# VinAIResearch/Point-Unet

Hardware: AMD Instinct MI355X
Metric: points_per_sec_forward (higher is better)
Workload: dtype f32

## Files before the change

point-unet_amd/csrc/common.h:

```cpp
#pragma once

#include <hip/hip_runtime.h>

#include <cstdarg>
#include <cstdint>
#include <cstdio>
#include <cstring>
#include <map>
#include <string>
#include <vector>

#include "../../include/pointseg.h"
#include "../../include/pointseg_train_ops.h"

namespace ps {

void set_error(const char* fmt, ...);

#define PS_HIP(expr)                                                                                  \
    do {                                                                                              \
        hipError_t _e = (expr);                                                                       \
        if (_e != hipSuccess) {                                                                       \
            ps::set_error("%s failed: %s (%s:%d)", #expr, hipGetErrorString(_e), __FILE__, __LINE__); \
            return PS_EHIP;                                                                           \
// ... 41 lines not shown
struct StageTimer {
    std::string name;
    std::vector<std::pair<hipEvent_t, hipEvent_t>> spans;
    int64_t launches = 0;
};

}

namespace ps {
struct PackJob {
    const float* w;
    int64_t sk, sn;
    int kind, cin, cout, ntb, p0, cblocks;
    void* out;
    int64_t total;
    bool same_key(const PackJob& o) const
    {
        return w == o.w && sk == o.sk && sn == o.sn && kind == o.kind && cin == o.cin && cout == o.cout && ntb == o.ntb && p0 == o.p0 && cblocks == o.cblocks;
    }
};
struct PackCache {
    int mode = 0;
    bool broken = false;
    size_t cursor = 0;
    std::vector<PackJob> jobs;
    std::vector<DevBuf> bufs;
    DevBuf table;
    int n_ops = 0, n_b3 = 0;
};
void* pack_slot(ps_context* c, const PackJob& key, size_t bytes, bool& launch);
int pack_cache_finish_recording(ps_context* c, PackCache& pc);
int pack_cache_replay(ps_context* c, PackCache& pc);
void pack_cache_clear(PackCache& pc);
int pack_batch_ops(ps_context* c, const PackJob* table, int n);
int pack_batch_b3(ps_context* c, const PackJob* table, int n);
}

namespace ps {
struct Tuning {
    double gemm32b_min_flops = 3e8;
    int gemm32b_rw = 0, gemm32b_cw = 0;
    bool gemm32_no_sk8 = false;
    bool att64_gemm = true;
    int att64_occ = 0;
    bool att_no_split = false;
    int64_t wgrad_b3_min_rows = 0;
    int64_t gemm_b3_min_rows = 0;
    int64_t wgrad_wgs = 512;
    bool bn_slice = false;
    bool inv_bucket = true;
    int inv_tile = 4096;
    bool gather_reduce_ordered = true;
    int maxpool_bwd_ordered = 1;
    bool train_act_bf16 = true;
    int train_att_gemm_split = -1;
    bool train_att_gemm = true;
    bool train_att128_fwd_gemm = true;
    bool train_fuse_residual = true;
    bool train_merge_syncbn = true;
    int convbn_max_c = 64;
    int convbn_rect_max = 1 << 30;
    bool wgrad_debug = false;
};
void tuning_from_env(Tuning& t);
}

struct ps_context {
    int device = 0;
    ps::Tuning tune;
    hipStream_t own_stream = nullptr;
    hipStream_t stream = nullptr;
    ps::Arena knn_arena;
    ps::Arena net_arena;
    ps::Arena sample_arena;
    ps::DevBuf stage_in;
    ps::DevBuf stage_out;
    ps::DevBuf red_ws;
    ps::DevBuf wgrad_ws;
    ps::PackCache* pack_cache = nullptr;
    ps::DevBuf ops_ring[4];
    int ops_ring_pos = 0;
    bool att_bf16x3 = true;
    bool regchain_b3 = true;
    bool att_lane = true;
    bool train_b3 = true;
    bool train_bf16 = false;
    bool train_act_bf16 = false;
    bool mid_lds_attr = false;
    size_t chain_lds_attr = 48 * 1024;
    std::map<const void*, size_t> regchain_lds_attr;
    bool deferred = false;
    int32_t* h_flags = nullptr;
    unsigned pending_mask = 0;
    uint64_t builds = 0;
    uint64_t samples = 0;
    uint64_t volume_samples = 0;
    uint64_t flag_serial[8] = {};
    int flag_kind[8] = {};
    int flag_slot = 0;
    int sticky_rc = 0;
    std::string sticky_msg;
    hipEvent_t flag_ev[8] = {};
    std::vector<char> host_ring[8];
    int ring_pos = 0;
    std::vector<char>& ring_next() { ring_pos = (ring_pos + 1) & 7; return host_ring[ring_pos]; }
    int check_deferred();
    int check_flag_slot(int s);
    int defer_status(const void* d_words, size_t bytes, int kind, uint64_t serial);
    struct PinSlot { void* p = nullptr; size_t cap = 0; hipEvent_t ev = nullptr; bool busy = false; };
    PinSlot pin[16];
    int pin_pos = 0;
    int upload_async(void* dst, const void* src, size_t bytes);
    bool timing = false;
    std::string timing_only;
    std::vector<ps::StageTimer> stages;
    std::vector<hipEvent_t> event_pool;
    size_t event_next = 0;
    int cur_stage = -1;
    hipEvent_t cur_start = nullptr;

    hipEvent_t get_event();
    void stage_begin(const char* name);
    void stage_end(int launches);
};

namespace ps {
struct Stage {
    ps_context* c;
    int n;
    bool on = false;
    Stage(ps_context* ctx, const char* name, int launches = 1) : c(ctx), n(launches)
    {
        on = c->timing && (c->timing_only.empty() || c->timing_only == name);
        if (on) c->stage_begin(name);
    }
    ~Stage()
    {
        if (on) c->stage_end(n);
    }
};

inline int ceil_div(int64_t a, int64_t b) { return (int)((a + b - 1) / b); }

inline uint64_t pyramid_stamp(const ps_pyramid* p)
{
    uint64_t h = 0x50535059524D4944ull ^ (uint64_t)p->B ^ ((uint64_t)p->K << 32) ^ ((uint64_t)p->num_layers << 48);
    for (int i = 0; i < p->num_layers && i < PS_MAX_LAYERS; ++i) {
        h = (h ^ (uint64_t)reinterpret_cast<uintptr_t>(p->sub_idx[i])) * 0x9E3779B97F4A7C15ull;
        h = (h ^ (uint64_t)reinterpret_cast<uintptr_t>(p->neigh_idx[i])) * 0x9E3779B97F4A7C15ull;
        h = (h ^ (uint64_t)reinterpret_cast<uintptr_t>(p->interp_idx[i])) * 0x9E3779B97F4A7C15ull;
        h = (h ^ (uint64_t)reinterpret_cast<uintptr_t>(p->order[i])) * 0x9E3779B97F4A7C15ull;
        h = (h ^ (uint64_t)p->n[i] ^ ((uint64_t)p->n[i + 1] << 32)) * 0x9E3779B97F4A7C15ull;
    }
    return h | 1ull;
}

int pool_max(ps_context* c, const float* feat, const int32_t* idx, const int32_t* order, float* out, int64_t B, int64_t n, int64_t m, int K, int ch,
             unsigned char* ties = nullptr);

int conv1x1(ps_context* c, const float* x, int64_t ldx, const float* w, bool w_transposed, const float* b, int64_t R, int64_t cin, int64_t cout, int leaky,
            int accumulate, float* y, int64_t ldy);
int att_bwd_split_impl(ps_context* c, const float* fl, int64_t ldl, const int32_t* idx, int64_t B, int64_t n_src, int64_t n_q, const float* fr,
                       int64_t ldr, const float* wfc, const float* dagg, int64_t K, int64_t d, float* dfl, int64_t lddl, float* dfr, int64_t lddr,
                       float* dwfc, float* dfl_rows, int64_t ld_rows, bool df_accum);
int random_sample_bwd_inv(ps_context* c, const float* dout, const float* out, const float* feature, const int32_t* pool_idx, const int32_t* offsets,
                          const int32_t* src, int64_t B, int64_t N, int64_t M, int64_t K, int64_t d, const uint8_t* ties, float* share_ws,
// ... 24 lines not shown
```

point-unet_amd/csrc/context.hip:

```cpp
#include "common.h"
#include "kdtree_build.h"

#include <cstdlib>

namespace ps {

static thread_local char g_err[512] = "";

void set_error(const char* fmt, ...)
{
    va_list ap;
    va_start(ap, fmt);
    vsnprintf(g_err, sizeof g_err, fmt, ap);
    va_end(ap);
}

int DevBuf::reserve(size_t bytes)
{
    if (bytes <= cap) return PS_OK;
    if (p) {
        hipError_t e = hipDeviceSynchronize();
        if (e != hipSuccess) {
            set_error("hipDeviceSynchronize failed: %s", hipGetErrorString(e));
            return PS_EHIP;
// ... 138 lines not shown
    }
    cur_start = get_event();
    if (cur_start) (void)hipEventRecord(cur_start, stream);
}

void ps_context::stage_end(int launches)
{
    hipEvent_t stop = get_event();
    if (stop) (void)hipEventRecord(stop, stream);
    if (cur_stage >= 0 && cur_start && stop) {
        stages[cur_stage].spans.push_back({cur_start, stop});
        stages[cur_stage].launches += launches;
    }
    cur_stage = -1;
}

extern "C" {

const char* ps_last_error(void) { return ps::g_err; }

}

namespace ps {
void tuning_from_env(Tuning& t)
{
#ifdef PS_TUNING_ENV
    auto num = [](const char* name, double& out) { const char* v = std::getenv(name); if (v && *v) { out = std::atof(v); return true; } return false; };
    auto flag = [&](const char* name, bool& b) { double v; if (num(name, v)) b = v != 0; };
    auto clampi = [&](const char* name, int64_t lo, int64_t hi, int64_t& x) { double v; if (num(name, v)) x = v < lo ? lo : (v > hi ? hi : (int64_t)v); };
    double v;
    if (num("PS_GEMM32B_MIN_FLOPS", v) && v >= 0) t.gemm32b_min_flops = v;
    if (num("PS_GEMM32B_RW", v) && (v == 1 || v == 2)) t.gemm32b_rw = (int)v;
    if (num("PS_GEMM32B_CW", v) && (v == 1 || v == 2)) t.gemm32b_cw = (int)v;
    t.gemm32_no_sk8 = std::getenv("PS_GEMM32_NO_SK8") != nullptr;
    flag("PS_ATT64_GEMM", t.att64_gemm);
    if (num("PS_ATT64_OCC", v) && (v == 1 || v == 2)) t.att64_occ = (int)v;
    t.att_no_split = std::getenv("PS_ATT_NO_SPLIT") != nullptr;
    clampi("PS_WGRAD_B3_MIN_ROWS", 0, 1ll << 40, t.wgrad_b3_min_rows);
    clampi("PS_GEMM_B3_MIN_ROWS", 0, 1ll << 40, t.gemm_b3_min_rows);
    clampi("PS_WGRAD_WGS", 64, 4096, t.wgrad_wgs);
    flag("PS_BN_SLICE", t.bn_slice);
    flag("PS_INV_BUCKET", t.inv_bucket);
    if (num("PS_INV_TILE", v) && (v == 4096 || v == 6144 || v == 8192)) t.inv_tile = (int)v;
    flag("PS_GATHER_REDUCE_ORDERED", t.gather_reduce_ordered);
    if (num("PS_MAXPOOL_BWD_ORDERED", v)) t.maxpool_bwd_ordered = v != 0;
    flag("PS_TRAIN_ACT_BF16", t.train_act_bf16);
    if (num("PS_TRAIN_ATT_GEMM_SPLIT", v)) t.train_att_gemm_split = v < 0 ? -1 : (v != 0);
    flag("PS_TRAIN_ATT_GEMM", t.train_att_gemm);
    flag("PS_TRAIN_ATT128_FWD_GEMM", t.train_att128_fwd_gemm);
    flag("PS_TRAIN_FUSE_RESIDUAL", t.train_fuse_residual);
    flag("PS_TRAIN_MERGE_SYNCBN", t.train_merge_syncbn);
    if (num("PS_CONVBN_MAX_C", v) && v >= 0 && v <= 4096) t.convbn_max_c = (int)v;
    if (num("PS_CONVBN_RECT_MAX", v) && v >= 0) t.convbn_rect_max = v > (double)(1 << 30) ? 1 << 30 : (int)v;
    t.wgrad_debug = std::getenv("PS_WGRAD_DEBUG") != nullptr;
#else
    (void)t;
#endif
}
}

extern "C" {
const char* ps_version(void) { return "pointseg-hip 0.1 gfx950"; }
int ps_abi_version(void) { return PS_ABI_VERSION; }

int ps_create(int device, ps_context** out)
{
    PS_CHECK(out != nullptr, "ps_create: out is NULL");
    int count = 0;
    PS_HIP(hipGetDeviceCount(&count));
    PS_CHECK(device >= 0 && device < count, "ps_create: device %d out of range (%d devices)", device, count);
    PS_HIP(hipSetDevice(device));
    ps_context* c = new ps_context();
    c->device = device;
    hipError_t e = hipStreamCreateWithFlags(&c->own_stream, hipStreamNonBlocking);
    if (e != hipSuccess) {
        delete c;
        ps::set_error("hipStreamCreate failed: %s", hipGetErrorString(e));
        return PS_EHIP;
    }
    c->stream = c->own_stream;
    ps::tuning_from_env(c->tune);
#ifdef PS_TUNING_ENV
    if (const char* v = std::getenv("PS_REGCHAIN_B3")) c->regchain_b3 = std::atof(v) != 0;
    if (const char* v = std::getenv("PS_ATT_LANE")) c->att_lane = std::atof(v) != 0;
#endif
    *out = c;
    return PS_OK;
}

int ps_destroy(ps_context* c)
{
    if (!c) return PS_OK;
    (void)hipSetDevice(c->device);
    (void)hipStreamSynchronize(c->stream);
    c->knn_arena.buf.release();
    c->net_arena.buf.release();
    c->sample_arena.buf.release();
    c->stage_in.release();
    c->stage_out.release();
    c->red_ws.release();
    c->wgrad_ws.release();
    for (auto& b : c->ops_ring) b.release();
    if (c->h_flags) (void)hipHostFree(c->h_flags);
    for (auto& e : c->flag_ev)
        if (e) (void)hipEventDestroy(e);
    for (auto& s : c->pin) {
        if (s.p) (void)hipHostFree(s.p);
        if (s.ev) (void)hipEventDestroy(s.ev);
    }
    for (hipEvent_t e : c->event_pool) (void)hipEventDestroy(e);
    if (c->own_stream) (void)hipStreamDestroy(c->own_stream);
    delete c;
    return PS_OK;
}

int ps_set_stream(ps_context* c, void* hip_stream)
{
    PS_CHECK(c != nullptr, "ps_set_stream: ctx is NULL");
    c->stream = static_cast<hipStream_t>(hip_stream);
    return PS_OK;
}

int ps_synchronize(ps_context* c)
{
    PS_CHECK(c != nullptr, "ps_synchronize: ctx is NULL");
    PS_HIP(hipStreamSynchronize(c->stream));
    return c->check_deferred();
}

int ps_set_train_gemm_bf16(ps_context* c, int on)
{
    PS_CHECK(c != nullptr, "ps_set_train_gemm_bf16: ctx is NULL");
    c->train_bf16 = on != 0;
    return PS_OK;
}

int ps_set_train_act_bf16(ps_context* c, int on)
{
    PS_CHECK(c != nullptr, "ps_set_train_act_bf16: ctx is NULL");
    c->train_act_bf16 = on != 0;
    return PS_OK;
}

int ps_set_train_gemm_b3(ps_context* c, int on)
{
    PS_CHECK(c != nullptr, "ps_set_train_gemm_b3: ctx is NULL");
    c->train_b3 = on != 0;
    return PS_OK;
}

int ps_set_att_bf16x3(ps_context* c, int on)
{
    PS_CHECK(c != nullptr, "ps_set_att_bf16x3: ctx is NULL");
    c->att_bf16x3 = on != 0;
    return PS_OK;
}

int ps_set_deferred_checks(ps_context* c, int on)
{
    PS_CHECK(c != nullptr, "ps_set_deferred_checks: ctx is NULL");
    if (on && !c->h_flags) PS_HIP(hipHostMalloc(reinterpret_cast<void**>(&c->h_flags), 8 * 4 * sizeof(int32_t)));
    if (!on && c->pending_mask) {
        PS_HIP(hipStreamSynchronize(c->stream));
        PS_TRY(c->check_deferred());
    }
    c->deferred = on != 0;
// ... 46 lines not shown
```

point-unet_amd/csrc/debug_hooks.h:

```cpp
#ifndef POINTSEG_DEBUG_H
#define POINTSEG_DEBUG_H
#include "../../include/pointseg.h"
#ifdef __cplusplus
extern "C" {
#endif
int ps_debug_knn_host(const float* support, const float* queries, int64_t B, int64_t n_support,
                      int64_t n_queries, int64_t K, int32_t* out_idx);
int ps_debug_kdtree_host(const float* support, int64_t n, int32_t* vind, int32_t* nodes, float* pts,
                         int32_t* root_depth, float* bbox);
int ps_debug_kdtree_device(ps_context* ctx, const float* support, int64_t n, int32_t* vind, int32_t* nodes,
                           float* pts, int32_t* root_depth, float* bbox);
#define PS_DEBUG_KDTREE_STATS 22
int ps_debug_kdtree_device_set(ps_context* ctx, const float* support, const int32_t* n, int64_t T, const int32_t* want_copy, int32_t* vind,
                               int32_t* nodes, float* pts, int32_t* fat, int32_t* root_depth, float* bbox, float* copy, int32_t* stats);
int ps_debug_pack_weights(const float* W, int cin, int cout, int ntb, float* out);
int ps_debug_pack_b3(const float* W, int cin, int cout, uint16_t* out);
int ps_debug_pack_b3_device(ps_context* ctx, const float* W, int cin, int cout, void* out);
int ps_debug_gemm32(ps_context* ctx, int split_bf16, const float* x1, int ld1, int c1, const int32_t* g1, const float* x2, int ld2, int c2,
                    const int32_t* g2, int gm, int gn, const float* W, const float* bias, int64_t R, int cout, int leaky, float* y, int ldy);
int ps_debug_gemm32_plan(ps_context* ctx, int split_bf16, int64_t R, int cin, int cout, int* out4);

typedef struct ps_debug_chain_layer {
    const float* W;
    const float* bias;
    int cin, cout, leaky;
    float* y;
    int ldy;
    const float* extra;
    int ld_extra, c_extra;
    const int32_t* extra_gather;
} ps_debug_chain_layer;
typedef struct ps_debug_chain_desc {
    int n_layers;
    ps_debug_chain_layer layer[4];
    const float* x1; const int32_t* g1; int ld1, c1, g1m, g1n;
    const float* x2; const int32_t* g2; int ld2, c2, g2m, g2n;
    int64_t R;
} ps_debug_chain_desc;
int ps_debug_chain(ps_context* ctx, const ps_debug_chain_desc* d, int form);
int ps_debug_chain_plan(const ps_debug_chain_desc* d, int* out4);
int ps_debug_chain_plan_prec(const ps_debug_chain_desc* d, int precision, int* out4);
int ps_debug_set_regchain_b3(ps_context* ctx, int on);
int ps_debug_set_att_lane(ps_context* ctx, int on);
int ps_debug_att_stage(ps_randla* net, int level, int stage, int form, const float* xyz, const int32_t* idx, const int32_t* order, const float* fg,
                       int64_t n_total, int64_t n_cloud, float* agg);
int ps_debug_att_form(ps_randla* net, int level, int stage, int k, int64_t n_total);
int ps_debug_dense_form(ps_randla* net, int which, int level, int64_t R);
int ps_debug_att_lane_pass_points(void);

int ps_debug_set_tuning(ps_context* ctx, const char* field, double value);
int ps_debug_get_tuning(ps_context* ctx, const char* field, double* value);
int ps_debug_tuning_fields(char* buf, int cap);
int ps_debug_volume_sample_args_size(void);

int64_t ps_debug_scan_words(int64_t n);
int64_t ps_debug_sort_words(int64_t n);
int ps_debug_scan_launches(int64_t n);
int ps_debug_sort_launches(int64_t n, int bits);
int ps_debug_scan_u32(ps_context* ctx, const uint32_t* in, uint32_t* out, int64_t n, uint32_t* work);
int ps_debug_sort_pairs(ps_context* ctx, int key_bytes, void* k0, void* k1, uint32_t* v0, uint32_t* v1, int64_t n, int bits, uint32_t* work,
                        int* which_out);
int ps_debug_reduce_partials(ps_context* ctx, int form, const void* part, int n_part, int nv, int n0, void* out0, void* out1);

#ifdef __cplusplus
}
#endif
#endif
```

point-unet_amd/csrc/debug_hooks.hip:

```cpp
#include "common.h"

#include <cstring>
#include <vector>
#include "kdtree_build.h"
#include "kdtree_host.h"
#include "rowgemm.h"
#include "attpool.h"
#include "b3_ops.h"
#include "debug_hooks.h"
#include "randla_net.h"
#include "reduce_partials.h"
#include "sortscan.h"

using namespace ps;

extern "C" int ps_debug_volume_sample_args_size(void) { return (int)sizeof(ps_volume_sample_args); }

extern "C" int ps_debug_pack_weights(const float* W, int cin, int cout, int ntb, float* out)
{
    PS_CHECK(W && out && (ntb == 1 || ntb == 2 || ntb == 4), "ps_debug_pack_weights: bad argument");
    pack_weights(W, cin, cout, ntb, out);
    return PS_OK;
}

// ... 169 lines not shown
    for (int i = 0; i < b.n; ++i) {
        const ps_debug_chain_layer& y = d->layer[i];
        PackedLinear& L = b.L[i];
        wp_off[i] = grow(L.packed_floats());
        const float* Wl = y.W;
        if (L.round) {
            wround.resize((size_t)y.cin * y.cout);
            for (size_t t = 0; t < wround.size(); ++t) wround[t] = b3_rounded(y.W[t]);
            Wl = wround.data();
        }
        pack_weights(Wl, y.cin, y.cout, L.ntb, host.data() + wp_off[i]);
        b_off[i] = grow((size_t)L.cout_pad());
        for (int k = 0; k < L.cout_pad(); ++k) host[b_off[i] + k] = (y.bias && k < y.cout) ? y.bias[k] : 0.f;
        wq_off[i] = 0;
        if (L.round) {
            wq_off[i] = grow(L.bf16_bytes() / 4);
            pack_weights_bf16(Wl, y.cin, y.cout, L.ntb, reinterpret_cast<uint16_t*>(host.data() + wq_off[i]));
            continue;
        }
        if (y.cin % 16 == 0) {
            wq_off[i] = grow(L.kperm_floats());
            pack_weights_kperm(y.W, y.cin, y.cout, L.ntb, host.data() + wq_off[i]);
        }
    }
    size_t total = (host.size() + 63) & ~size_t(63);
    for (int i = 0; i < b.n; ++i) {
        tmp_off[i] = total;
        if (form == 3 && !d->layer[i].y) total += ((size_t)d->R * d->layer[i].cout + 63) & ~size_t(63);
    }
    float* dev = nullptr;
    PS_HIP(hipMalloc(reinterpret_cast<void**>(&dev), total * sizeof(float)));
    int rc = PS_OK;
    if (hipMemcpyAsync(dev, host.data(), host.size() * sizeof(float), hipMemcpyHostToDevice, c->stream) != hipSuccess) {
        set_error("ps_debug_chain: upload failed");
        rc = PS_EHIP;
    }
    for (int i = 0; i < b.n; ++i) {
        b.L[i].wp = dev + wp_off[i];
        b.L[i].bias = dev + b_off[i];
        if (b.L[i].round) b.L[i].wb = dev + wq_off[i];
        else b.L[i].wq = wq_off[i] ? dev + wq_off[i] : nullptr;
    }
    if (rc == PS_OK) {
        if (form == 0) {
            ChainCache cache;
            if (rowchain_fits(b.steps, b.n, b.s1, b.s2)) rc = rowchain(c, b.steps, b.n, b.s1, b.s2, d->R, &cache);
            else { set_error("ps_debug_chain: the chain fits neither chain kernel (channels above %d, mismatched, or a gathered extra)", kChainMaxC); rc = PS_EINVAL; }
            (void)hipStreamSynchronize(c->stream);
            cache.clear();
        } else if (form == 1) {
            if (regchain_fits(b.steps, b.n, b.s1, b.s2)) rc = regchain(c, b.steps, b.n, b.s1, b.s2, d->R, nullptr);
            else { set_error("ps_debug_chain: not one of regchain's compiled chain shapes"); rc = PS_EINVAL; }
        } else if (form == 2) {
            if (rowchain_lds_plan(b.steps, b.n, b.s1, b.s2, d->R).form == 2) rc = rowchain_lds(c, b.steps, b.n, b.s1, b.s2, d->R);
            else { set_error("ps_debug_chain: the chain does not fit the LDS-staged kernel (channels above %d, mismatched, or a gathered extra)", kChainMaxC); rc = PS_EINVAL; }
        } else {
            RowSrc in1 = b.s1, in2 = b.s2;
            for (int i = 0; i < b.n && rc == PS_OK; ++i) {
                const ChainStep& st = b.steps[i];
                if (i > 0) {
                    in2 = RowSrc();
                    if (st.extra.x) in2 = st.extra;
                }
                float* out = st.y ? st.y : dev + tmp_off[i];
                const int ldo = st.y ? st.ldy : b.L[i].cout;
                rc = rowgemm(c, b.L[i], in1, in2, d->R, out, ldo);
                in1 = RowSrc();
                in1.x = out; in1.ld = ldo; in1.c = b.L[i].cout;
            }
        }
    }
    (void)hipStreamSynchronize(c->stream);
    (void)hipFree(dev);
    return rc;
}

extern "C" int ps_debug_set_regchain_b3(ps_context* c, int on)
{
    PS_CHECK(c && (on == 0 || on == 1), "ps_debug_set_regchain_b3: bad argument");
    c->regchain_b3 = on != 0;
    return PS_OK;
}

extern "C" int ps_debug_set_att_lane(ps_context* c, int on)
{
    PS_CHECK(c && (on == 0 || on == 1), "ps_debug_set_att_lane: bad argument");
    c->att_lane = on != 0;
    return PS_OK;
}

extern "C" int ps_debug_att_stage(ps_randla* net, int level, int stage, int form, const float* xyz, const int32_t* idx, const int32_t* order,
                                  const float* fg, int64_t n_total, int64_t n_cloud, float* agg)
{
    PS_CHECK(net && xyz && idx && fg && agg, "ps_debug_att_stage: NULL argument");
    PS_CHECK(net->have_weights, "ps_debug_att_stage: weights not set");
    PS_CHECK(level >= 0 && level < net->cfg.num_layers && (stage == 1 || stage == 2) && form >= 0 && form <= 5, "ps_debug_att_stage: bad level / stage / form");
    PS_CHECK(n_total >= 0 && n_cloud >= 1 && n_total % n_cloud == 0, "ps_debug_att_stage: n_total must be a whole number of clouds");
    ps_context* c = net->ctx;
    PS_HIP(hipSetDevice(c->device));
    const bool one_plane = form == 5 || (form == 0 && net->precision == 2);
    const NetImages* images = net;
    if (one_plane && net->enc[level].has_p32) {
        PS_TRY(randla_bf16_images(net));
        images = net->bf16.get();
    }
    const EncLevel& e = images->enc[level];
    const int d = e.d, h = d / 2;
    const bool use_g = d >= 64;
    AttStage s;
    s.one_plane = one_plane ? 1 : 0;
    s.xyz = xyz; s.idx = idx; s.order = order; s.fg = fg; s.lfa1 = &e.lfa1; s.agg = agg;
    s.n_total = n_total; s.n_cloud = n_cloud; s.d = d; s.k = net->cfg.k_n; s.ldf = use_g ? h + d : h;
    s.p32 = e.has_p32 ? &e.p32 : nullptr;
    s.lfa2 = stage == 2 ? &e.lfa2 : nullptr;
    s.wbot = use_g ? (stage == 1 ? &e.bot1 : &e.bot2) : nullptr;
    s.wfull = use_g ? nullptr : (stage == 1 ? &e.full1 : &e.full2);
    s.lane = stage == 1 ? e.lane1 : e.lane2;
    int rc = PS_EINVAL;
    if (form == 4) rc = att_lane_stage(c, s);
    else if (form == 0) rc = att_pool_stage(c, s);
    else if (form == 1 && att_pool32b_fits(s)) rc = att_pool32b_stage(c, s);
    else if (form == 2 && att_pool32_fits(s)) rc = att_pool32_stage(c, s);
    else if (form == 3) rc = att_pool16_stage(c, s);
    else if (form == 5 && att_pool32b_fits(s)) rc = att_pool32b_stage(c, s);
    else set_error("ps_debug_att_stage: the level (d = %d, %lld rows) does not fit the 32x32 form %d", d, (long long)n_total, form);
    (void)hipStreamSynchronize(c->stream);
    return rc;
}

extern "C" int ps_debug_att_form(ps_randla* net, int level, int stage, int k, int64_t n_total)
{
    if (!net || !net->have_weights || level < 0 || level >= net->cfg.num_layers || (stage != 1 && stage != 2) || k < 1 || n_total < 0) {
        set_error("ps_debug_att_form: bad argument");
        return -1;
    }
    const EncLevel& e = net->enc[level];
    const int d = e.d, h = d / 2;
    const bool use_g = d >= 64;
    AttStage s;
    s.lfa1 = &e.lfa1; s.lfa2 = stage == 2 ? &e.lfa2 : nullptr;
    s.wbot = use_g ? (stage == 1 ? &e.bot1 : &e.bot2) : nullptr;
    s.wfull = use_g ? nullptr : (stage == 1 ? &e.full1 : &e.full2);
    s.lane = stage == 1 ? e.lane1 : e.lane2;
    s.p32 = e.has_p32 ? &e.p32 : nullptr;
    s.n_total = n_total; s.n_cloud = n_total; s.d = d; s.k = k; s.ldf = use_g ? h + d : h;
    s.one_plane = net->precision == 2 ? 1 : 0;
    return att_pool_form(net->ctx, s);
}

extern "C" int ps_debug_dense_form(ps_randla* net, int which, int level, int64_t R)
{
    if (!net || !net->have_weights || which < 0 || which > 4 || level < 0 || level >= net->cfg.num_layers || R < 1) {
        set_error("ps_debug_dense_form: bad argument");
        return -1;
    }
    const NetImages* I = net;
    if (net->precision == 2) {
        if (randla_bf16_images(net) != PS_OK) return -1;
        I = net->bf16.get();
    }
    const EncLevel& e = I->enc[level];
    const PackedLinear& L = which == 0 ? e.att1mlp : which == 1 ? e.att2mlp : which == 2 ? e.mlp2sc : which == 3 ? I->decoder0 : I->dec[level];
    static const float4 aligned = {0.f, 0.f, 0.f, 0.f};
    RowSrc s1, s2;
    s1.x = &aligned.x; s1.c = s1.ld = L.cin;
    if (which == 2) { s1.c = s1.ld = e.d; s2.x = &aligned.x; s2.c = s2.ld = e.d_in; }
// ... 246 lines not shown
```

point-unet_amd/csrc/regchain.hip:

```cpp
#include <algorithm>
#include <type_traits>

#include "b3_ops.h"
#include "mfma_tile.h"
#include "rowgemm.h"

namespace ps {

struct RcLayer {
    const float* wp;
    const float* bias;
    float* y;
    const float* ex;
    int ca, cb;
    int ta, tb;
    int cout, ot;
    int ks, ntb;
    int ldy, ldex, leaky;
    int w_off, b_off;
};
struct RcArgs {
    const float* x1; const int32_t* g1; int ld1, g1m, g1n;
    const float* x2; const int32_t* g2; int ld2, g2m, g2n;
    int n, R;
// ... 160 lines not shown
        }
        f32x4 acc[OT];
#pragma unroll
        for (int to = 0; to < OT; ++to) acc[to] = f32x4{0.f, 0.f, 0.f, 0.f};
        if constexpr (L > 0) __builtin_amdgcn_sched_barrier(0);
        P::template mma<IT, OT>(acc, act, lds + y.w_off, lane);
        const bool vy = y.y && (y.cout & 3) == 0 && (y.ldy & 3) == 0 && (reinterpret_cast<uintptr_t>(y.y) & 15) == 0;
#pragma unroll
        for (int to = 0; to < OT; ++to) {
            const int ch = to * 16 + 4 * g;
            const float4 b = *reinterpret_cast<const float4*>(lds + y.b_off + ch);
            float v[4] = {acc[to][0] + b.x, acc[to][1] + b.y, acc[to][2] + b.z, acc[to][3] + b.w};
#pragma unroll
            for (int q = 0; q < 4; ++q) {
                if (y.leaky) v[q] = leaky02(v[q]);
                act[to][q] = v[q];
            }
            if (y.y && ok) {
                float* o = y.y + (size_t)row * y.ldy + ch;
                if (vy) {
                    if (to + 1 < OT || ch < y.cout) *reinterpret_cast<float4*>(o) = make_float4(v[0], v[1], v[2], v[3]);
                } else {
#pragma unroll
                    for (int q = 0; q < 4; ++q)
                        if (to + 1 < OT || ch + q < y.cout) o[q] = v[q];
                }
            }
        }
        rc_layer<S, P, L + 1>(a, act, lds, lane, g, row, rr, ok);
    }
}

template <class P>
__device__ __forceinline__ void rc_stage(const RcArgs& a, float* dst)
{
    for (int l = 0; l < a.n; ++l) {
        const RcLayer& y = a.l[l];
        P::stage(y, dst);
        for (int e = threadIdx.x; e < y.ot * 16; e += P::kThreads) dst[y.b_off + e] = e < y.cout ? y.bias[e] : 0.f;
    }
}

template <class P>
__global__ __launch_bounds__(P::kThreads) void rc_pack_kernel(RcArgs a, float* out) { rc_stage<P>(a, out); }

template <class S, class P>
__global__ __launch_bounds__(P::kThreads) void regchain_kernel(RcArgs a)
{
    extern __shared__ __attribute__((aligned(16))) float rc_lds[];
    constexpr int MT = S::maxt(), WAVES = P::kThreads / 64;
    const int wave = threadIdx.x >> 6, lane = threadIdx.x & 63;
    const int p = lane & 15, g = lane >> 4;
    if (a.image) {
        for (int i = threadIdx.x; i < a.image_floats / 4; i += P::kThreads) reinterpret_cast<float4*>(rc_lds)[i] = reinterpret_cast<const float4*>(a.image)[i];
    } else {
        rc_stage<P>(a, rc_lds);
    }
    __syncthreads();

    const bool v1 = (a.l[0].ca & 3) == 0 && (a.ld1 & 3) == 0 && (reinterpret_cast<uintptr_t>(a.x1) & 15) == 0;
    const bool v2 = (a.l[0].cb & 3) == 0 && (a.ld2 & 3) == 0 && (reinterpret_cast<uintptr_t>(a.x2) & 15) == 0;
    const int stride = gridDim.x * WAVES;
    auto load_inputs = [&](int tile, float (&dst)[MT][4]) {
        const int rr = min(tile * 16 + p, a.R - 1);
        const int s1 = a.g1 ? (a.g1m ? (rr / a.g1m) * a.g1n : 0) + a.g1[rr] : rr;
        rc_load<0, S::A0>(dst, a.x1 + (size_t)s1 * a.ld1, a.l[0].ca, v1, g);
        if constexpr (S::B[0] > 0) {
            const int s2 = a.g2 ? (a.g2m ? (rr / a.g2m) * a.g2n : 0) + a.g2[rr] : rr;
            rc_load<S::A0, S::B[0]>(dst, a.x2 + (size_t)s2 * a.ld2, a.l[0].cb, v2, g);
        }
    };
    int tile = blockIdx.x * WAVES + wave;
    float act[MT][4], nxt[MT][4];
    if (tile * 16 < a.R) load_inputs(tile, nxt);
    for (; tile * 16 < a.R; tile += stride) {
#pragma unroll
        for (int t = 0; t < S::IN(0); ++t)
#pragma unroll
            for (int q = 0; q < 4; ++q) act[t][q] = nxt[t][q];
        if ((tile + stride) * 16 < a.R) load_inputs(tile + stride, nxt);
        const int row = tile * 16 + p;
        rc_layer<S, P, 0>(a, act, rc_lds, lane, g, row, min(row, a.R - 1), row < a.R);
    }
}

static inline int rc_tiles(int c) { return (c + 15) / 16; }

using RcFc0 = RcShape<2, 1, 0, 1, 0, 1>;
using RcEnc0 = RcShape<2, 1, 0, 1, 1, 2>;
using RcOne0 = RcShape<1, 1, 0, 1>;
using RcPair1 = RcShape<2, 2, 0, 2, 0, 4>;
using RcPair1b = RcShape<2, 4, 0, 2, 0, 4>;
using RcEnc1 = RcShape<2, 4, 0, 4, 2, 8>;
using RcPair2 = RcShape<2, 8, 0, 4, 0, 8>;
using RcHead = RcShape<4, 2, 2, 2, 0, 4, 0, 2, 0, 1>;

template <class S>
static bool rc_matches(const RcArgs& a)
{
    if (a.n != S::N) return false;
    for (int l = 0; l < S::N; ++l)
        if (a.l[l].ta != S::A(l) || a.l[l].tb != S::B[l] || a.l[l].ot != S::O[l]) return false;
    return true;
}

template <class S>
constexpr bool rc_even_inputs()
{
    for (int l = 0; l < S::N; ++l)
        if (S::IN(l) & 1) return false;
    return true;
}
template <class S>
constexpr bool kRcSplit = std::is_same<S, RcHead>::value || std::is_same<S, RcEnc1>::value || std::is_same<S, RcPair1>::value ||
                          std::is_same<S, RcPair1b>::value;

template <class S>
constexpr bool kRcOnePlane = kRcSplit<S> || std::is_same<S, RcPair2>::value;

static size_t rc_layout(RcArgs& a, int pair_floats)
{
    int off = 0;
    for (int i = 0; i < a.n; ++i) {
        RcLayer& y = a.l[i];
        y.w_off = off; off += y.ot * (y.ta + y.tb) * pair_floats;
        y.b_off = off; off += y.ot * 16;
    }
    return (size_t)off * sizeof(float);
}

static bool rc_build(const ChainStep* steps, int n_steps, const RowSrc& s1, const RowSrc& s2, RcArgs& a, size_t& lds_bytes, bool& rounded)
{
    rounded = false;
    if (n_steps < 1 || n_steps > kChainMaxSteps) return false;
    a = RcArgs{};
    a.x1 = s1.x; a.g1 = s1.gather; a.ld1 = s1.ld; a.g1m = s1.gm; a.g1n = s1.gn;
    a.x2 = s2.x; a.g2 = s2.gather; a.ld2 = s2.ld; a.g2m = s2.gm; a.g2n = s2.gn;
    a.n = n_steps;
    int prev = 0;
    for (int i = 0; i < n_steps; ++i) {
        const PackedLinear* L = steps[i].L;
        if (!L || !L->wp || !L->bias) return false;
        if (steps[i].extra.x && (i == 0 || steps[i].extra.gather)) return false;
        RcLayer& y = a.l[i];
        y.wp = L->wp; y.bias = L->bias; y.y = steps[i].y; y.ldy = steps[i].ldy;
        y.ex = i > 0 ? steps[i].extra.x : nullptr; y.ldex = steps[i].extra.ld;
        y.ca = i == 0 ? s1.c : prev;
        y.cb = i == 0 ? s2.c : (steps[i].extra.x ? steps[i].extra.c : 0);
        if (y.ca + y.cb != L->cin) return false;
        y.ta = rc_tiles(y.ca); y.tb = rc_tiles(y.cb);
        y.cout = L->cout; y.ot = rc_tiles(L->cout);
        y.ks = L->ks; y.ntb = L->ntb; y.leaky = L->leaky;
        prev = L->cout;
    }
    int n_round = 0;
    for (int i = 0; i < n_steps; ++i) n_round += steps[i].L->round != 0;
    if (n_round) {
        if (n_round != n_steps) return false;
        rounded = true;
        lds_bytes = rc_layout(a, RcB1::kPairFloats);
        return rc_matches<RcPair1>(a) || rc_matches<RcPair1b>(a) || rc_matches<RcEnc1>(a) || rc_matches<RcPair2>(a) || rc_matches<RcHead>(a);
    }
    lds_bytes = rc_layout(a, RcF32::kPairFloats);
    return rc_matches<RcFc0>(a) || rc_matches<RcEnc0>(a) || rc_matches<RcOne0>(a) || rc_matches<RcPair1>(a) || rc_matches<RcPair1b>(a) ||
           rc_matches<RcEnc1>(a) || rc_matches<RcPair2>(a) || rc_matches<RcHead>(a);
}

bool regchain_fits(const ChainStep* steps, int n_steps, const RowSrc& s1, const RowSrc& s2)
{
    RcArgs a;
    size_t lds = 0;
    bool rounded = false;
    return rc_build(steps, n_steps, s1, s2, a, lds, rounded);
}

static int rc_blocks(int64_t R, size_t lds_bytes, int waves)
{
    const int64_t tiles = (R + 15) / 16;
    const int per_cu = std::max(1, std::min(16 / waves, (int)(160 * 1024 / std::max<size_t>(lds_bytes, 1))));
    return (int)std::max<int64_t>(1, std::min<int64_t>((tiles + waves - 1) / waves, 256 * per_cu));
}

ChainPlan regchain_plan(const ChainStep* steps, int n_steps, const RowSrc& s1, const RowSrc& s2, int64_t R)
{
    ChainPlan p;
    RcArgs a;
    bool rounded = false;
    if (!rc_build(steps, n_steps, s1, s2, a, p.lds_bytes, rounded)) return ChainPlan();
    p.form = rounded ? 3 : 1;
    p.blocks = rc_blocks(R, p.lds_bytes, (rounded ? RcB1::kThreads : RcF32::kThreads) / 64);
    return p;
}

template <class S, class P>
static int rc_run(ps_context* c, RcArgs& a, ChainCache* cache)
{
    constexpr int policy = std::is_same<P, RcB3>::value ? 1 : (std::is_same<P, RcB1>::value ? 2 : 0);
    const size_t lds_bytes = rc_layout(a, P::kPairFloats);
    if (cache) {
        ChainCache::Entry* hit = nullptr;
        for (auto& e : cache->entries)
            if (e.wp0 == a.l[0].wp && e.wp_last == a.l[a.n - 1].wp && e.n == a.n && e.ca == a.l[0].ca && e.cb == a.l[0].cb && e.policy == policy) hit = &e;
        if (!hit) {
            cache->entries.emplace_back();
            hit = &cache->entries.back();
            hit->wp0 = a.l[0].wp; hit->wp_last = a.l[a.n - 1].wp; hit->n = a.n; hit->ca = a.l[0].ca; hit->cb = a.l[0].cb; hit->policy = policy;
            PS_TRY(hit->img.reserve(lds_bytes));
            hipLaunchKernelGGL(rc_pack_kernel<P>, dim3(1), dim3(P::kThreads), 0, c->stream, a, hit->img.as<float>());
            PS_HIP(hipGetLastError());
        }
        a.image = hit->img.as<float>();
        a.image_floats = (int)(lds_bytes / sizeof(float));
    }
    size_t& have = c->regchain_lds_attr[reinterpret_cast<const void*>(regchain_kernel<S, P>)];
    if (lds_bytes > 48 * 1024 && lds_bytes > have) {
        PS_HIP(hipFuncSetAttribute(reinterpret_cast<const void*>(regchain_kernel<S, P>), hipFuncAttributeMaxDynamicSharedMemorySize, (int)lds_bytes));
        have = lds_bytes;
    }
    hipLaunchKernelGGL((regchain_kernel<S, P>), dim3(rc_blocks(a.R, lds_bytes, P::kThreads / 64)), dim3(P::kThreads), lds_bytes, c->stream, a);
    PS_HIP(hipGetLastError());
    return PS_OK;
}

template <class S>
static int rc_route(ps_context* c, RcArgs& a, ChainCache* cache, bool rounded)
{
    if constexpr (kRcOnePlane<S>) {
        static_assert(rc_even_inputs<S>(), "the one-plane policy takes its K axis in pairs of 16-channel tiles");
        if (rounded) return rc_run<S, RcB1>(c, a, cache);
    }
    if constexpr (kRcSplit<S>) {
        static_assert(rc_even_inputs<S>(), "the split-bf16 policy takes its K axis in pairs of 16-channel tiles");
        if (c->regchain_b3) return rc_run<S, RcB3>(c, a, cache);
    }
    return rc_run<S, RcF32>(c, a, cache);
}

int regchain(ps_context* c, const ChainStep* steps, int n_steps, const RowSrc& s1, const RowSrc& s2, int64_t R, ChainCache* cache)
{
    if (R <= 0) return PS_OK;
    RcArgs a;
    size_t lds_bytes = 0;
    bool rounded = false;
    PS_CHECK(rc_build(steps, n_steps, s1, s2, a, lds_bytes, rounded), "regchain: not one of the compiled chain shapes");
    PS_CHECK(R < (int64_t)1 << 31, "regchain: too many rows");
    a.R = (int)R;
    if (rc_matches<RcFc0>(a)) return rc_route<RcFc0>(c, a, cache, rounded);
    if (rc_matches<RcEnc0>(a)) return rc_route<RcEnc0>(c, a, cache, rounded);
    if (rc_matches<RcOne0>(a)) return rc_route<RcOne0>(c, a, cache, rounded);
    if (rc_matches<RcPair1>(a)) return rc_route<RcPair1>(c, a, cache, rounded);
    if (rc_matches<RcPair1b>(a)) return rc_route<RcPair1b>(c, a, cache, rounded);
    if (rc_matches<RcEnc1>(a)) return rc_route<RcEnc1>(c, a, cache, rounded);
    if (rc_matches<RcPair2>(a)) return rc_route<RcPair2>(c, a, cache, rounded);
    return rc_route<RcHead>(c, a, cache, rounded);
}

}
```

Baseline: 198.3 million.

## Add shape-specialized planned regchain kernels with compile-time channels, strides and 32-bit offsets

Adds a planned variant of the register-chain MLP kernel that bakes in channel counts, leading dimensions, gather flags and store flags for each known network layer chain. Each chain gets a compile-time plan, which lets loads and stores use float4 with 32-bit byte offsets, full tiles run without bounds checks, and gather division use a magic-multiply reciprocal. The next tile's inputs are prefetched while the current one computes. Any chain that does not match a plan falls back to the generic kernel. When no cache is supplied, the path builds a local image and synchronizes the stream, and it adds more template instantiations.

New measurement: 197.0 million. About the same (-0.6%).

```diff
diff --git a/point-unet_amd/csrc/common.h b/point-unet_amd/csrc/common.h
--- a/point-unet_amd/csrc/common.h
+++ b/point-unet_amd/csrc/common.h
@@ -147,6 +147,7 @@
     int ops_ring_pos = 0;
     bool att_bf16x3 = true;
     bool regchain_b3 = true;
+    bool regchain_plan = true;
     bool att_lane = true;
     bool train_b3 = true;
     bool train_bf16 = false;
diff --git a/point-unet_amd/csrc/context.hip b/point-unet_amd/csrc/context.hip
--- a/point-unet_amd/csrc/context.hip
+++ b/point-unet_amd/csrc/context.hip
@@ -244,6 +244,7 @@
     ps::tuning_from_env(c->tune);
 #ifdef PS_TUNING_ENV
     if (const char* v = std::getenv("PS_REGCHAIN_B3")) c->regchain_b3 = std::atof(v) != 0;
+    if (const char* v = std::getenv("PS_REGCHAIN_PLAN")) c->regchain_plan = std::atof(v) != 0;
     if (const char* v = std::getenv("PS_ATT_LANE")) c->att_lane = std::atof(v) != 0;
 #endif
     *out = c;
diff --git a/point-unet_amd/csrc/debug_hooks.h b/point-unet_amd/csrc/debug_hooks.h
--- a/point-unet_amd/csrc/debug_hooks.h
+++ b/point-unet_amd/csrc/debug_hooks.h
@@ -41,6 +41,7 @@
 int ps_debug_chain_plan(const ps_debug_chain_desc* d, int* out4);
 int ps_debug_chain_plan_prec(const ps_debug_chain_desc* d, int precision, int* out4);
 int ps_debug_set_regchain_b3(ps_context* ctx, int on);
+int ps_debug_set_regchain_plan(ps_context* ctx, int on);
 int ps_debug_set_att_lane(ps_context* ctx, int on);
 int ps_debug_att_stage(ps_randla* net, int level, int stage, int form, const float* xyz, const int32_t* idx, const int32_t* order, const float* fg,
                        int64_t n_total, int64_t n_cloud, float* agg);
diff --git a/point-unet_amd/csrc/debug_hooks.hip b/point-unet_amd/csrc/debug_hooks.hip
--- a/point-unet_amd/csrc/debug_hooks.hip
+++ b/point-unet_amd/csrc/debug_hooks.hip
@@ -275,6 +275,13 @@
     return PS_OK;
 }
 
+extern "C" int ps_debug_set_regchain_plan(ps_context* c, int on)
+{
+    PS_CHECK(c && (on == 0 || on == 1), "ps_debug_set_regchain_plan: bad argument");
+    c->regchain_plan = on != 0;
+    return PS_OK;
+}
+
 extern "C" int ps_debug_set_att_lane(ps_context* c, int on)
 {
     PS_CHECK(c && (on == 0 || on == 1), "ps_debug_set_att_lane: bad argument");
diff --git a/point-unet_amd/csrc/regchain.hip b/point-unet_amd/csrc/regchain.hip
--- a/point-unet_amd/csrc/regchain.hip
+++ b/point-unet_amd/csrc/regchain.hip
@@ -266,6 +266,163 @@
         const int row = tile * 16 + p;
         rc_layer<S, P, 0>(a, act, rc_lds, lane, g, row, min(row, a.R - 1), row < a.R);
     }
+}
+
+struct RpSrc { int c, ld, gathered; };
+struct RpLayer { int cout, cex, ldex, leaky, store, ldy; };
+
+struct RpArgs {
+    const float* x[2];
+    const int32_t* g[2];
+    uint32_t gn[2], gmul[2], gsh[2];
+    const float* ex[kChainMaxSteps];
+    float* y[kChainMaxSteps];
+    const float* image;
+    uint32_t R;
+    int multi;
+};
+
+template <class T>
+__device__ __forceinline__ T rp_ld(const void* base, uint32_t off) { return *reinterpret_cast<const T*>(static_cast<const char*>(base) + off); }
+template <class T>
+__device__ __forceinline__ void rp_st(void* base, uint32_t off, const T& v) { *reinterpret_cast<T*>(static_cast<char*>(base) + off) = v; }
+
+template <int T0, int C, int LD, int MT>
+__device__ __forceinline__ void rp_load(float (&dst)[MT][4], const float* x, uint32_t off, int g)
+{
+    constexpr int NT = (C + 15) / 16;
+#pragma unroll
+    for (int t = 0; t < NT; ++t) {
+        if constexpr ((C & 3) == 0 && (LD & 3) == 0) {
+            float4 v = make_float4(0.f, 0.f, 0.f, 0.f);
+            if (16 * t + 16 <= C || 16 * t + 4 * g < C) v = rp_ld<float4>(x, off + 64 * t);
+            dst[T0 + t][0] = v.x; dst[T0 + t][1] = v.y; dst[T0 + t][2] = v.z; dst[T0 + t][3] = v.w;
+        } else {
+#pragma unroll
+            for (int q = 0; q < 4; ++q) {
+                dst[T0 + t][q] = 0.f;
+                if (16 * t + 16 <= C || 16 * t + 4 * g + q < C) dst[T0 + t][q] = rp_ld<float>(x, off + 64 * t + 4 * q);
+            }
+        }
+    }
+}
+
+template <class PL, int W, bool MULTI>
+__device__ __forceinline__ uint32_t rp_src_off(const RpArgs& a, uint32_t row, int g)
+{
+    constexpr RpSrc s = W ? PL::s2 : PL::s1;
+    uint32_t r = row;
+    if constexpr (s.gathered != 0) {
+        r = (uint32_t)rp_ld<int32_t>(a.g[W], row * 4);
+        if constexpr (MULTI) r += (__umulhi(row, a.gmul[W]) >> a.gsh[W]) * a.gn[W];
+    }
+    return r * (uint32_t)(s.ld * 4) + 16 * g;
+}
+
+template <class PL, bool MULTI, int MT>
+__device__ __forceinline__ void rp_load_inputs(const RpArgs& a, float (&dst)[MT][4], uint32_t row, int g)
+{
+    using S = typename PL::S;
+    rp_load<0, PL::s1.c, PL::s1.ld>(dst, a.x[0], rp_src_off<PL, 0, MULTI>(a, row, g), g);
+    if constexpr (S::B[0] > 0) rp_load<S::A0, PL::s2.c, PL::s2.ld>(dst, a.x[1], rp_src_off<PL, 1, MULTI>(a, row, g), g);
+}
+
+template <class S, class P>
+constexpr int rp_w_off(int l)
+{
+    int off = 0;
+    for (int i = 0; i < l; ++i) off += S::O[i] * S::IN(i) * P::kPairFloats + S::O[i] * 16;
+    return off;
+}
+template <class S, class P>
+constexpr int rp_b_off(int l) { return rp_w_off<S, P>(l) + S::O[l] * S::IN(l) * P::kPairFloats; }
+
+template <class PL, class P, int L, bool FULL>
+__device__ __forceinline__ void rp_layer(const RpArgs& a, float (&act)[PL::S::maxt()][4], const float* lds, int lane, int g, uint32_t row, uint32_t rr, bool ok)
+{
+    using S = typename PL::S;
+    if constexpr (L < S::N) {
+        constexpr int IT = S::IN(L), OT = S::O[L], TA = S::A(L), TB = S::B[L];
+        constexpr RpLayer Y = PL::l[L];
+        if constexpr (L > 0 && TB > 0) rp_load<TA, Y.cex, Y.ldex>(act, a.ex[L], rr * (uint32_t)(Y.ldex * 4) + 16 * g, g);
+        f32x4 acc[OT];
+#pragma unroll
+        for (int to = 0; to < OT; ++to) acc[to] = f32x4{0.f, 0.f, 0.f, 0.f};
+        if constexpr (L > 0) __builtin_amdgcn_sched_barrier(0);
+        P::template mma<IT, OT>(acc, act, lds + rp_w_off<S, P>(L), lane);
+        const uint32_t yoff = row * (uint32_t)(Y.ldy * 4) + 16 * g;
+#pragma unroll
+        for (int to = 0; to < OT; ++to) {
+            const int ch = to * 16 + 4 * g;
+            const float4 b = *reinterpret_cast<const float4*>(lds + rp_b_off<S, P>(L) + ch);
+            float v[4] = {acc[to][0] + b.x, acc[to][1] + b.y, acc[to][2] + b.z, acc[to][3] + b.w};
+#pragma unroll
+            for (int q = 0; q < 4; ++q) {
+                if constexpr (Y.leaky != 0) v[q] = leaky02(v[q]);
+                act[to][q] = v[q];
+            }
+            if constexpr (Y.store != 0) {
+                if (FULL || ok) {
+                    if constexpr ((Y.cout & 3) == 0) {
+                        if (16 * to + 16 <= Y.cout || ch < Y.cout) rp_st(a.y[L], yoff + 64 * to, make_float4(v[0], v[1], v[2], v[3]));
+                    } else {
+                        static_assert(Y.cout == 2 && Y.ldy == 2, "a planned layer stores multiples of four channels, or two");
+                        if (g == 0) rp_st(a.y[L], yoff, make_float2(v[0], v[1]));
+                    }
+                }
+            }
+        }
+        rp_layer<PL, P, L + 1, FULL>(a, act, lds, lane, g, row, rr, ok);
+    }
+}
+
+template <class PL, class P, bool MULTI>
+__device__ __forceinline__ void rp_tiles(const RpArgs& a, const float* lds)
+{
+    using S = typename PL::S;
+    constexpr int MT = S::maxt(), WAVES = P::kThreads / 64;
+    const int wave = threadIdx.x >> 6, lane = threadIdx.x & 63;
+    const int g = lane >> 4;
+    const uint32_t p = lane & 15, R = a.R, stride = gridDim.x * WAVES;
+    uint32_t tile = blockIdx.x * WAVES + wave;
+    if (tile * 16 >= R) return;
+    float act[MT][4], nxt[MT][4];
+    auto prefetch = [&](uint32_t t) {
+        if (t * 16 + 16 <= R) rp_load_inputs<PL, MULTI>(a, nxt, t * 16 + p, g);
+        else if (t * 16 < R) rp_load_inputs<PL, MULTI>(a, nxt, min(t * 16 + p, R - 1), g);
+    };
+    auto take = [&]() {
+#pragma unroll
+        for (int t = 0; t < S::IN(0); ++t)
+#pragma unroll
+            for (int q = 0; q < 4; ++q) act[t][q] = nxt[t][q];
+    };
+    prefetch(tile);
+    for (; tile * 16 + 16 <= R; tile += stride) {
+        take();
+        prefetch(tile + stride);
+        const uint32_t row = tile * 16 + p;
+        rp_layer<PL, P, 0, true>(a, act, lds, lane, g, row, row, true);
+    }
+    if (tile * 16 < R) {
+        take();
+        const uint32_t row = tile * 16 + p;
+        rp_layer<PL, P, 0, false>(a, act, lds, lane, g, row, min(row, R - 1), row < R);
+    }
+}
+
+template <class PL, class P>
+__global__ __launch_bounds__(P::kThreads) void regchain_plan_kernel(RpArgs a)
+{
+    extern __shared__ __attribute__((aligned(16))) float rc_lds[];
+    using S = typename PL::S;
+    constexpr int kImageFloats = rp_w_off<S, P>(S::N);
+    for (int i = threadIdx.x; i < kImageFloats / 4; i += P::kThreads) reinterpret_cast<float4*>(rc_lds)[i] = reinterpret_cast<const float4*>(a.image)[i];
+    __syncthreads();
+    if constexpr (PL::s1.gathered != 0 || PL::s2.gathered != 0) {
+        if (a.multi) return rp_tiles<PL, P, true>(a, rc_lds);
+    }
+    rp_tiles<PL, P, false>(a, rc_lds);
 }
 
 static inline int rc_tiles(int c) { return (c + 15) / 16; }
@@ -376,31 +533,196 @@
     return p;
 }
 
+template <class P>
+static int rc_cached_image(ps_context* c, RcArgs& a, ChainCache& cache, size_t lds_bytes)
+{
+    constexpr int policy = std::is_same<P, RcB3>::value ? 1 : (std::is_same<P, RcB1>::value ? 2 : 0);
+    ChainCache::Entry* hit = nullptr;
+    for (auto& e : cache.entries)
+        if (e.wp0 == a.l[0].wp && e.wp_last == a.l[a.n - 1].wp && e.n == a.n && e.ca == a.l[0].ca && e.cb == a.l[0].cb && e.policy == policy) hit = &e;
+    if (!hit) {
+        cache.entries.emplace_back();
+        hit = &cache.entries.back();
+        hit->wp0 = a.l[0].wp; hit->wp_last = a.l[a.n - 1].wp; hit->n = a.n; hit->ca = a.l[0].ca; hit->cb = a.l[0].cb; hit->policy = policy;
+        PS_TRY(hit->img.reserve(lds_bytes));
+        hipLaunchKernelGGL(rc_pack_kernel<P>, dim3(1), dim3(P::kThreads), 0, c->stream, a, hit->img.as<float>());
+        PS_HIP(hipGetLastError());
+    }
+    a.image = hit->img.as<float>();
+    a.image_floats = (int)(lds_bytes / sizeof(float));
+    return PS_OK;
+}
+
+static int rc_raise_lds(ps_context* c, const void* kernel, size_t lds_bytes)
+{
+    size_t& have = c->regchain_lds_attr[kernel];
+    if (lds_bytes > 48 * 1024 && lds_bytes > have) {
+        PS_HIP(hipFuncSetAttribute(kernel, hipFuncAttributeMaxDynamicSharedMemorySize, (int)lds_bytes));
+        have = lds_bytes;
+    }
+    return PS_OK;
+}
+
+struct RpFc0in7 {
+    using S = RcFc0;
+    static constexpr RpSrc s1{7, 7, 0}, s2{0, 0, 0};
+    static constexpr RpLayer l[kChainMaxSteps] = {{8, 0, 0, 1, 1, 8}, {8, 0, 0, 1, 1, 8}};
+};
+struct RpFc0in4 {
+    using S = RcFc0;
+    static constexpr RpSrc s1{4, 4, 0}, s2{0, 0, 0};
+    static constexpr RpLayer l[kChainMaxSteps] = {{8, 0, 0, 1, 1, 8}, {8, 0, 0, 1, 1, 8}};
+};
+struct RpOne0 {
+    using S = RcOne0;
+    static constexpr RpSrc s1{16, 16, 0}, s2{0, 0, 0};
+    static constexpr RpLayer l[kChainMaxSteps] = {{8, 0, 0, 1, 1, 8}};
+};
+struct RpEnc0 {
+    using S = RcEnc0;
+    static constexpr RpSrc s1{16, 16, 0}, s2{0, 0, 0};
+    static constexpr RpLayer l[kChainMaxSteps] = {{16, 0, 0, 1, 0, 0}, {32, 8, 8, 1, 1, 32}};
+};
+struct RpPair1 {
+    using S = RcPair1;
+    static constexpr RpSrc s1{32, 32, 0}, s2{0, 0, 0};
+    static constexpr RpLayer l[kChainMaxSteps] = {{32, 0, 0, 1, 1, 96}, {64, 0, 0, 0, 1, 96}};
+};
+struct RpPair1b {
+    using S = RcPair1b;
+    static constexpr RpSrc s1{64, 64, 0}, s2{0, 0, 0};
+    static constexpr RpLayer l[kChainMaxSteps] = {{32, 0, 0, 1, 1, 96}, {64, 0, 0, 0, 1, 96}};
+};
+struct RpEnc1 {
+    using S = RcEnc1;
+    static constexpr RpSrc s1{64, 64, 0}, s2{0, 0, 0};
+    static constexpr RpLayer l[kChainMaxSteps] = {{64, 0, 0, 1, 0, 0}, {128, 32, 32, 1, 1, 128}};
+};
+struct RpPair2 {
+    using S = RcPair2;
+    static constexpr RpSrc s1{128, 128, 0}, s2{0, 0, 0};
+    static constexpr RpLayer l[kChainMaxSteps] = {{64, 0, 0, 1, 1, 192}, {128, 0, 0, 0, 1, 192}};
+};
+struct RpHead4 {
+    using S = RcHead;
+    static constexpr RpSrc s1{32, 32, 0}, s2{32, 32, 1};
+    static constexpr RpLayer l[kChainMaxSteps] = {{32, 0, 0, 1, 0, 0}, {64, 0, 0, 1, 0, 0}, {32, 0, 0, 1, 0, 0}, {4, 0, 0, 0, 1, 4}};
+};
+struct RpHead2 {
+    using S = RcHead;
+    static constexpr RpSrc s1{32, 32, 0}, s2{32, 32, 1};
+    static constexpr RpLayer l[kChainMaxSteps] = {{32, 0, 0, 1, 0, 0}, {64, 0, 0, 1, 0, 0}, {32, 0, 0, 1, 0, 0}, {2, 0, 0, 0, 1, 2}};
+};
+template <class... PLs>
+struct RpList {};
+template <class S> struct RpOf { using plans = RpList<>; };
+template <> struct RpOf<RcFc0> { using plans = RpList<RpFc0in7, RpFc0in4>; };
+template <> struct RpOf<RcOne0> { using plans = RpList<RpOne0>; };
+template <> struct RpOf<RcEnc0> { using plans = RpList<RpEnc0>; };
+template <> struct RpOf<RcPair1> { using plans = RpList<RpPair1>; };
+template <> struct RpOf<RcPair1b> { using plans = RpList<RpPair1b>; };
+template <> struct RpOf<RcEnc1> { using plans = RpList<RpEnc1>; };
+template <> struct RpOf<RcPair2> { using plans = RpList<RpPair2>; };
+template <> struct RpOf<RcHead> { using plans = RpList<RpHead4, RpHead2>; };
+
+static bool rp_aligned16(const void* p) { return (reinterpret_cast<uintptr_t>(p) & 15) == 0; }
+static bool rp_below_4g(int64_t rows, int ld) { return rows * ld * 4 < ((int64_t)1 << 32); }
+
+template <class PL>
+static bool rp_matches(const RcArgs& a)
+{
+    using S = typename PL::S;
+    if (!rc_matches<S>(a) || a.R >= (1 << 30)) return false;
+    const RpSrc src[2] = {PL::s1, PL::s2};
+    const float* x[2] = {a.x1, a.x2};
+    const int32_t* gt[2] = {a.g1, a.g2};
+    const int c[2] = {a.l[0].ca, a.l[0].cb}, ld[2] = {a.ld1, a.ld2}, gm[2] = {a.g1m, a.g2m}, gn[2] = {a.g1n, a.g2n};
+    for (int w = 0; w < 2; ++w) {
+        const RpSrc& s = src[w];
+        if (c[w] != s.c) return false;
+        if (!s.c) continue;
+        if (ld[w] != s.ld || (gt[w] != nullptr) != (s.gathered != 0)) return false;
+        if (((s.c | s.ld) & 3) == 0 && !rp_aligned16(x[w])) return false;
+        int64_t rows = a.R;
+        if (s.gathered) {
+            if (gm[w] < 2 || gn[w] < 1) return false;
+            rows = ((int64_t)a.R + gm[w] - 1) / gm[w] * gn[w];
+        }
+        if (!rp_below_4g(rows, s.ld)) return false;
+    }
+    for (int l = 0; l < S::N; ++l) {
+        const RcLayer& y = a.l[l];
+        const RpLayer& Y = PL::l[l];
+        if (y.cout != Y.cout || (y.leaky != 0) != (Y.leaky != 0) || (y.y != nullptr) != (Y.store != 0)) return false;
+        if (Y.store && (y.ldy != Y.ldy || !rp_aligned16(y.y) || !rp_below_4g(a.R, Y.ldy))) return false;
+        if (l > 0) {
+            if (y.cb != Y.cex) return false;
+            if (Y.cex && (y.ldex != Y.ldex || !rp_aligned16(y.ex) || !rp_below_4g(a.R, Y.ldex))) return false;
+        }
+    }
+    return true;
+}
+
+static void rp_reciprocal(uint32_t d, uint32_t& mul, uint32_t& sh)
+{
+    uint32_t l = 1;
+    while (((uint64_t)1 << l) < d) ++l;
+    mul = (uint32_t)((((uint64_t)1 << (31 + l)) + d - 1) / d);
+    sh = l - 1;
+}
+
+template <class PL, class P>
+static int rp_run(ps_context* c, RcArgs& a, ChainCache* cache)
+{
+    using S = typename PL::S;
+    const size_t lds_bytes = rc_layout(a, P::kPairFloats);
+    constexpr size_t image_bytes = sizeof(float) * rp_w_off<S, P>(S::N);
+    PS_CHECK(lds_bytes == image_bytes, "regchain: the planned kernel's LDS layout is not rc_layout's");
+    ChainCache local;
+    int rc = rc_cached_image<P>(c, a, cache ? *cache : local, lds_bytes);
+    const void* kernel = reinterpret_cast<const void*>(regchain_plan_kernel<PL, P>);
+    if (rc == PS_OK) rc = rc_raise_lds(c, kernel, lds_bytes);
+    if (rc == PS_OK) {
+        RpArgs r{};
+        r.x[0] = a.x1; r.x[1] = a.x2; r.g[0] = a.g1; r.g[1] = a.g2;
+        const int gm[2] = {a.g1m, a.g2m}, gn[2] = {a.g1n, a.g2n};
+        for (int w = 0; w < 2; ++w)
+            if (r.g[w]) {
+                r.gn[w] = (uint32_t)gn[w];
+                rp_reciprocal((uint32_t)gm[w], r.gmul[w], r.gsh[w]);
+                if (a.R > gm[w]) r.multi = 1;
+            }
+        for (int l = 0; l < S::N; ++l) { r.ex[l] = a.l[l].ex; r.y[l] = a.l[l].y; }
+        r.image = a.image;
+        r.R = (uint32_t)a.R;
+        hipLaunchKernelGGL((regchain_plan_kernel<PL, P>), dim3(rc_blocks(a.R, lds_bytes, P::kThreads / 64)), dim3(P::kThreads), lds_bytes, c->stream, r);
+        if (hipGetLastError() != hipSuccess) { set_error("regchain: the planned kernel did not launch"); rc = PS_EHIP; }
+    }
+    if (!cache) {
+        (void)hipStreamSynchronize(c->stream);
+        local.clear();
+    }
+    return rc;
+}
+
+template <class P, class... PLs>
+static bool rp_try(RpList<PLs...>, ps_context* c, RcArgs& a, ChainCache* cache, int& rc)
+{
+    return ((rp_matches<PLs>(a) ? (rc = rp_run<PLs, P>(c, a, cache), true) : false) || ...);
+}
+
 template <class S, class P>
 static int rc_run(ps_context* c, RcArgs& a, ChainCache* cache)
 {
-    constexpr int policy = std::is_same<P, RcB3>::value ? 1 : (std::is_same<P, RcB1>::value ? 2 : 0);
+    if constexpr (!std::is_same<P, RcB1>::value) {
+        int rc = PS_OK;
+        if (c->regchain_plan && rp_try<P>(typename RpOf<S>::plans(), c, a, cache, rc)) return rc;
+    }
     const size_t lds_bytes = rc_layout(a, P::kPairFloats);
     if (cache) {
-        ChainCache::Entry* hit = nullptr;
-        for (auto& e : cache->entries)
-            if (e.wp0 == a.l[0].wp && e.wp_last == a.l[a.n - 1].wp && e.n == a.n && e.ca == a.l[0].ca && e.cb == a.l[0].cb && e.policy == policy) hit = &e;
-        if (!hit) {
-            cache->entries.emplace_back();
-            hit = &cache->entries.back();
-            hit->wp0 = a.l[0].wp; hit->wp_last = a.l[a.n - 1].wp; hit->n = a.n; hit->ca = a.l[0].ca; hit->cb = a.l[0].cb; hit->policy = policy;
-            PS_TRY(hit->img.reserve(lds_bytes));
-            hipLaunchKernelGGL(rc_pack_kernel<P>, dim3(1), dim3(P::kThreads), 0, c->stream, a, hit->img.as<float>());
-            PS_HIP(hipGetLastError());
-        }
-        a.image = hit->img.as<float>();
-        a.image_floats = (int)(lds_bytes / sizeof(float));
-    }
-    size_t& have = c->regchain_lds_attr[reinterpret_cast<const void*>(regchain_kernel<S, P>)];
-    if (lds_bytes > 48 * 1024 && lds_bytes > have) {
-        PS_HIP(hipFuncSetAttribute(reinterpret_cast<const void*>(regchain_kernel<S, P>), hipFuncAttributeMaxDynamicSharedMemorySize, (int)lds_bytes));
-        have = lds_bytes;
-    }
+        PS_TRY(rc_cached_image<P>(c, a, *cache, lds_bytes));
+    }
+    PS_TRY(rc_raise_lds(c, reinterpret_cast<const void*>(regchain_kernel<S, P>), lds_bytes));
     hipLaunchKernelGGL((regchain_kernel<S, P>), dim3(rc_blocks(a.R, lds_bytes, P::kThreads / 64)), dim3(P::kThreads), lds_bytes, c->stream, a);
     PS_HIP(hipGetLastError());
     return PS_OK;
```
